# yuhang1008/WildGS-SLAM-Blackwell

Measured on AMD Instinct MI355X. Metric: rasterised Gaussians/s fwd+bwd @1M pts 1080p; PSNR vs ref, higher is better.
Workload: dtype f32; 1 GPU; configs[2]: 1000000 Gaussians, 1920x1080, SH3, single-view fwd+bwd, pose grad on; gaussians=1000000, image=1920x1080, sh_degree=3, num_rendered=13015374, parallelism=dp1 (keyframe views), dp_exchange=none

## Files before the change

wildgs-slam-blackwell_amd/csrc/capi.hip:

```cpp
#include <cstdarg>
#include <cstdio>
#include <cstdlib>
#include <cstring>
#include <vector>

#include <immintrin.h>

#include "wgsr.h"
#include "wgsr_common.h"
#include "wgsr_internal.h"

namespace wgsr {

namespace {
thread_local char g_err[1024] = "";

struct HostCounters {
  uint32_t* buf = nullptr;
  hipEvent_t ev = nullptr;
  hipStream_t side = nullptr;
  hipEvent_t pre = nullptr;
  uint4* mbox = nullptr;
  uint32_t seq = 0;
};
constexpr int kMaxDevices = 64;
int device_slot() {
  int dev = 0;
  return hipGetDevice(&dev) == hipSuccess && dev >= 0 && dev < kMaxDevices ? dev : -1;
}
struct BinningGuess {
  int P = -1, W = 0, H = 0, bshift = -1;
  size_t bytes = 0;
};
BinningGuess& binning_guess() {
  thread_local BinningGuess g[kMaxDevices];
  const int dev = device_slot();
  return g[dev < 0 ? 0 : dev];
}

bool publish_counts() {
  static const bool on = [] {
    const char* e = getenv("WGSR_PUBLISH_COUNTS");
    return !(e && e[0] == '0');
  }();
  return on;
}

HostCounters& host_counters() {
  thread_local HostCounters per_dev[kMaxDevices];
  const int dev = device_slot();
  HostCounters& hc = per_dev[dev < 0 ? 0 : dev];
  if (!hc.buf) {
    void* p = nullptr;
    if (hipHostMalloc(&p, kCounterBytes, hipHostMallocDefault) != hipSuccess) p = nullptr;
    hc.buf = static_cast<uint32_t*>(p);
    if (hipEventCreateWithFlags(&hc.ev, hipEventDisableTiming) != hipSuccess) hc.ev = nullptr;
    if (hipStreamCreateWithFlags(&hc.side, hipStreamNonBlocking) != hipSuccess) hc.side = nullptr;
    if (hc.side && hipEventCreateWithFlags(&hc.pre, hipEventDisableTiming) != hipSuccess) hc.pre = nullptr;
    if (!hc.pre) hc.side = nullptr;
    void* m = nullptr;
    if (publish_counts() &&
        hipHostMalloc(&m, 256, hipHostMallocCoherent | hipHostMallocMapped) == hipSuccess) {
      hc.mbox = static_cast<uint4*>(m);
      *hc.mbox = make_uint4(0u, 0u, 0u, 0u);
    }
  }
  return hc;
}

struct DevCounters {
  uint32_t* buf = nullptr;
  int parity = 0;
  bool failed = false;
};
bool bds_emit(int bshift) { return bshift <= 1; }

DevCounters* dev_counters(hipStream_t s) {
  thread_local DevCounters per_dev[kMaxDevices];
  const int dev = device_slot();
  if (dev < 0) return nullptr;
  DevCounters& dc = per_dev[dev];
  if (!dc.buf && !dc.failed) {
    void* p = nullptr;
    if (hipMalloc(&p, 2 * kCounterBytes) != hipSuccess || hipMemsetAsync(p, 0, 2 * kCounterBytes, s) != hipSuccess) {
      dc.failed = true;
      return nullptr;
    }
    dc.buf = static_cast<uint32_t*>(p);
  }
  return dc.buf ? &dc : nullptr;
}

}

int set_error(int code, const char* fmt, ...) {
  va_list ap;
  va_start(ap, fmt);
  vsnprintf(g_err, sizeof(g_err), fmt, ap);
  va_end(ap);
  return code;
}

int num_bits(uint32_t n) {
  int b = 0;
  while (b < 32 && (1ull << b) < n) ++b;
  return b;
}

namespace {

enum Stage { kStPreprocess, kStDepthSort, kStOffsetsScan, kStDuplicate, kStTileSort, kStRanges, kStRenderFwd,
             kStRenderBwd, kStGaussBwd, kStDistCuda2, kNumStages };
const char* const kStageNames[] = {"preprocess", "depth_sort", "offsets_scan", "duplicate", "tile_sort",
                                   "ranges",     "render_fwd", "render_bwd",   "gauss_bwd", "dist_cuda2"};
static_assert(kNumStages == WGSR_NUM_STAGES && sizeof(kStageNames) / sizeof(kStageNames[0]) == kNumStages,
              "Stage, kStageNames and WGSR_NUM_STAGES list the same stages in the same order");
struct Prof {
  uint32_t mask = 0;
  struct Rec { int stage; hipEvent_t a, b; };
  std::vector<Rec> recs;
  std::vector<hipEvent_t> pool;
  double ms[WGSR_NUM_STAGES] = {};
  int64_t count[WGSR_NUM_STAGES] = {};
  hipEvent_t get() {
    if (!pool.empty()) { hipEvent_t e = pool.back(); pool.pop_back(); return e; }
    hipEvent_t e = nullptr;
    if (hipEventCreate(&e) != hipSuccess) return nullptr;
    return e;
  }
  void flush() {
    for (auto& r : recs) {
      float t = 0.f;
      if (hipEventSynchronize(r.b) == hipSuccess && hipEventElapsedTime(&t, r.a, r.b) == hipSuccess) {
        ms[r.stage] += t;
        count[r.stage] += 1;
      }
      pool.push_back(r.a);
      pool.push_back(r.b);
    }
    recs.clear();
  }
};
Prof g_prof;

struct StageTimer {
  Stage stage;
  hipStream_t s;
  hipEvent_t a = nullptr;
  StageTimer(Stage st, hipStream_t str) : stage(st), s(str) {
    if (((g_prof.mask >> st) & 1u) && (a = g_prof.get()) && hipEventRecord(a, s) != hipSuccess) a = nullptr;
  }
  ~StageTimer() {
    if (!a) return;
    hipEvent_t b = g_prof.get();
    if (b && hipEventRecord(b, s) == hipSuccess) g_prof.recs.push_back({stage, a, b});
    else g_prof.pool.push_back(a);
  }
};

struct Grid {
  int gx, gy, nt;
  explicit Grid(const wgsr_raster_args& a)
      : gx((a.W + kTile - 1) / kTile), gy((a.H + kTile - 1) / kTile), nt(gx * gy) {}
};

int sort_bits(int n) { return num_bits((uint32_t)n) > 0 ? num_bits((uint32_t)n) : 1; }

constexpr int kDefaultBinShift = 2;
constexpr int kSmallFrameTiles = 2048;
int bin_shift(const wgsr_raster_args& a) {
  const char* e = getenv("WGSR_BIN_SHIFT");
  const Grid g(a);
  int sh = e ? atoi(e) : (g.nt <= kSmallFrameTiles ? 1 : kDefaultBinShift);
  sh = sh < 0 ? 0 : (sh > kMaxBinShift ? kMaxBinShift : sh);
  return sh > 0 && g.nt > 65535 ? 0 : sh;
}
enum class DepthSched { kBins, kGlobal, kFull };
DepthSched depth_schedule(int bshift) {
  const char* e = getenv("WGSR_DEPTH_SORT");
  if (e && strcmp(e, "full") == 0) return DepthSched::kFull;
  if (!bshift || (e && strcmp(e, "global") == 0)) return DepthSched::kGlobal;
  return DepthSched::kBins;
}
size_t bin_depth_max_avg() {
  const char* e = getenv("WGSR_BIN_DEPTH_MAX_AVG");
  return e ? (size_t)strtoull(e, nullptr, 10) : (size_t)6144;
}
constexpr int kDepthBits = 32;
constexpr bool kFullDepthInAlt = ((kDepthBits + 7) / 8) % 2 == 1;
thread_local int64_t g_depth_order_off = -1;

int validate(const wgsr_raster_args* a) {
  if (!a) return set_error(WGSR_EINVAL, "null args");
  if (a->P < 0) return set_error(WGSR_EINVAL, "means3D must have dimensions (num_points, 3)");
  if (a->W <= 0 || a->H <= 0) return set_error(WGSR_EINVAL, "image size must be positive (got %dx%d)", a->W, a->H);
  if (a->P == 0) return WGSR_OK;
  if (!a->means3D || !a->opacities || !a->bg || !a->viewmatrix || !a->projmatrix || !a->campos)
    return set_error(WGSR_EINVAL, "missing required tensor");
  if ((a->shs == nullptr) == (a->colors == nullptr))
    return set_error(WGSR_EINVAL, "Please provide excatly one of either SHs or precomputed colors!");
  const bool sr = a->scales && a->rotations;
  if (sr == (a->cov3D_precomp != nullptr))
    return set_error(WGSR_EINVAL,
                     "Please provide exactly one of either scale/rotation pair or precomputed 3D covariance!");
  if (a->shs && (a->M <= 0 || a->D < 0 || a->D > 3 || (a->D + 1) * (a->D + 1) > a->M))
    return set_error(WGSR_EINVAL, "invalid SH configuration (degree %d, %d coefficients)", a->D, a->M);
  const Grid g(*a);
  if (g.gx > 65535 || g.gy > 65535) return set_error(WGSR_EINVAL, "image too large");
  return WGSR_OK;
}

#define HIPCHK(expr)                                                                          \
  do {                                                                                        \
    hipError_t _e = (expr);                                                                   \
    if (_e != hipSuccess) return set_error(WGSR_EHIP, "%s: %s", #expr, hipGetErrorString(_e)); \
  } while (0)

#define STAGE(a, s, expr)                   \
  do {                                      \
    HIPCHK(expr);                           \
    if ((a).debug) {                        \
      HIPCHK(hipStreamSynchronize(s));      \
      HIPCHK(hipGetLastError());            \
    }                                       \
  } while (0)

void* call_alloc(wgsr_alloc_fn fn, void* ctx, size_t bytes) { return fn ? fn(ctx, bytes) : nullptr; }

struct Fwd {
  const wgsr_raster_args& a;
  hipStream_t s;
  Grid grid; GeomLayout GL; ImageLayout IL;
  int bshift;
  float *out_color, *out_depth, *out_opacity;
  int32_t* n_touched;
  void *geom = nullptr, *image = nullptr;
  uint32_t* counter = nullptr;
  template <typename T> T* g(size_t off) const { return at<T>(geom, off); }
  template <typename T> T* im(size_t off) const { return at<T>(image, off); }
  int alloc(wgsr_alloc_fn geom_alloc, wgsr_alloc_fn image_alloc, void* ctx) {
    if (!(geom = call_alloc(geom_alloc, ctx, GL.total)))
      return set_error(WGSR_EALLOC, "geometry buffer allocation failed");
    if (!(image = call_alloc(image_alloc, ctx, IL.total)))
      return set_error(WGSR_EALLOC, "image buffer allocation failed");
    return WGSR_OK;
  }
};

struct BinningPlan {
  BinLayout BL;
  size_t lists_bytes, bds_bytes, total;
  BinningPlan(size_t N_rect, size_t N_bin, int bshift, bool bin_depth)
      : BL(N_rect), lists_bytes(bshift ? align256(4 * (N_bin << (2 * bshift))) : 0),
        bds_bytes(bin_depth ? align256(16 * N_bin) : 0), total(BL.total + lists_bytes + bds_bytes) {}
};

struct Counts {
  size_t N_rect, N, N_bin;
  uint32_t flags;
  bool published;
};

int start_counts_readback(const Fwd& f, bool bin_depth, HostCounters& hc, PublishJob* pub) {
  if (!hc.buf || !hc.ev) return set_error(WGSR_EHIP, "pinned counter buffer / event allocation failed");
  if (bin_depth && hc.mbox) {
    *pub = PublishJob{f.counter, hc.mbox, hc.seq = (hc.seq % 0xFFFFFFu) + 1u};
  } else if (hc.side && !bin_depth) {
    HIPCHK(hipEventRecord(hc.pre, f.s));
    HIPCHK(hipStreamWaitEvent(hc.side, hc.pre, 0));
    HIPCHK(hipMemcpyAsync(hc.buf, f.counter, kCounterBytes, hipMemcpyDeviceToHost, hc.side));
    HIPCHK(hipEventRecord(hc.ev, hc.side));
  } else {
    HIPCHK(hipMemcpyAsync(hc.buf, f.counter, kCounterBytes, hipMemcpyDeviceToHost, f.s));
    HIPCHK(hipEventRecord(hc.ev, f.s));
  }
  return WGSR_OK;
}

int wait_counts(const Fwd& f, HostCounters& hc, const PublishJob& pub, Counts* c) {
  if (!pub.counter) {
    HIPCHK(hipEventSynchronize(hc.ev));
  } else {
    uint4 rec = make_uint4(0u, 0u, 0u, 0u);
    auto poll = [&]() {
      asm volatile("" ::: "memory");
      const __m128i v = _mm_load_si128(reinterpret_cast<const __m128i*>(const_cast<const uint4*>(hc.mbox)));
      _mm_storeu_si128(reinterpret_cast<__m128i*>(&rec), v);
      return (rec.x >> 8) == pub.seq;
    };
    uint32_t polls = 0;
    while (!poll()) {
      _mm_pause();
      if ((++polls & 1023u) == 0) {
        const hipError_t q = hipStreamQuery(f.s);
        if (q == hipErrorNotReady) continue;
        HIPCHK(q);
        bool seen = false;
        for (int k = 0; k < (1 << 16) && !(seen = poll()); ++k) _mm_pause();
        if (seen) break;
        hc.mbox = nullptr;
        break;
      }
    }
    if (hc.mbox && !(rec.x & 0x80u)) {
      *c = Counts{rec.y, rec.z, rec.w, rec.x & 0x7Fu, true};
      return WGSR_OK;
    }
    HIPCHK(hipMemcpyAsync(hc.buf, f.counter, kCounterBytes, hipMemcpyDeviceToHost, f.s));
    HIPCHK(hipStreamSynchronize(f.s));
  }
  *c = Counts{0, 0, 0, hc.buf[1], false};
  const uint64_t* partial = reinterpret_cast<const uint64_t*>(hc.buf + 4);
  for (int i = 0; i < kRectPairLanes; ++i) {
    c->N_rect += partial[i];
    c->N += partial[kRectPairLanes + i];
    c->N_bin += partial[2 * kRectPairLanes + i];
  }
  return WGSR_OK;
}

int read_depth_range(const Fwd& f, HostCounters& hc, const Counts& c, uint32_t* hi, uint32_t* nlo) {
  if (c.published) {
    HIPCHK(hipMemcpyAsync(hc.buf, f.counter, kCounterBytes, hipMemcpyDeviceToHost, f.s));
    HIPCHK(hipStreamSynchronize(f.s));
  }
  const uint32_t* rw = hc.buf + kDepthRangeOffset / 4;
  *hi = *nlo = 0;
  for (int i = 0; i < kRectPairLanes; ++i) {
    *hi = rw[i] > *hi ? rw[i] : *hi;
    *nlo = rw[kRectPairLanes + i] > *nlo ? rw[kRectPairLanes + i] : *nlo;
  }
  return WGSR_OK;
}

ZeroJob preprocess_zero_job(const Fwd& f, const DevCounters* dc, DepthSched sched) {
  const size_t P = (size_t)f.a.P;
  ZeroJob zj{};
  auto add = [&](void* p, size_t words) {
    if (words) { zj.p[zj.count] = static_cast<float*>(p); zj.n[zj.count++] = words; }
  };
  if (dc) add(dc->buf + (size_t)(dc->parity ^ 1) * (kCounterBytes / 4), kCounterBytes / 4);
  size_t sup_off = depth_sort_sup_offset_words(P);
  const size_t sup_words = sched == DepthSched::kFull     ? sort_sup_words(P, 0, kDepthBits, &sup_off)
                           : sched == DepthSched::kGlobal ? depth_sort_sup_words(P)
                                                          : 0;
  add(f.g<uint32_t>(f.GL.hist) + sup_off, sup_words);
  if (f.bshift) add(f.g<float>(f.GL.bsup), 2 * kScanSupStride * packed_scan_supers(P));
  return zj;
}

int queue_depth_sort(const Fwd& f, bool full, bool zero_sup, const uint32_t** depth_order) {
  const GeomLayout& GL = f.GL;
  const size_t P = (size_t)f.a.P;
  uint32_t *dkey = f.g<uint32_t>(GL.dkey), *dkey_alt = f.g<uint32_t>(GL.dkey_alt), *dval = f.g<uint32_t>(GL.dval),
           *dval_alt = f.g<uint32_t>(GL.dval_alt), *hist = f.g<uint32_t>(GL.hist);
  StageTimer T(kStDepthSort, f.s);
  if (full) {
    const bool sup_zeroed = sort_sup_words(P, 0, kDepthBits, nullptr) != 0;
    bool in_alt = false;
    STAGE(f.a, f.s, radix_sort_pairs(dkey, dkey_alt, dval, dval_alt, true, P, 0, kDepthBits, hist,
                                     f.g<uint32_t>(GL.totals), f.s, &in_alt, nullptr, nullptr, sup_zeroed));
    if (in_alt != kFullDepthInAlt) return set_error(WGSR_EHIP, "internal: depth sort parity");
    *depth_order = kFullDepthInAlt ? dval_alt : dval;
    return WGSR_OK;
  }
  if (zero_sup)
    HIPCHK(hipMemsetAsync(hist + depth_sort_sup_offset_words(P), 0, 4 * depth_sort_sup_words(P), f.s));
  STAGE(f.a, f.s, launch_depth_sort(dkey, dkey_alt, dval, dval_alt, P, f.counter + kDepthRangeOffset / 4,
                                    f.counter + 2, hist, f.s));
  *depth_order = dval_alt;
  return WGSR_OK;
}

int queue_scan(const Fwd& f, const uint32_t* depth_order, const PublishJob& pj) {
  const GeomLayout& GL = f.GL;
  StageTimer T(kStOffsetsScan, f.s);
  if (f.bshift) {
    STAGE(f.a, f.s, packed_scan_blocks(f.g<uint32_t>(GL.tb), 1, depth_order, (size_t)f.a.P, f.g<uint32_t>(GL.bsum),
// ... 454 lines not shown
```

wildgs-slam-blackwell_amd/csrc/raster_fwd.hip:

```cpp
#include <stdlib.h>
#include <string.h>

#include <type_traits>

#include "wgsr_common.h"
#include "wgsr_internal.h"

namespace wgsr {

namespace {

constexpr float SH_C0 = 0.28209479177387814f;
constexpr float SH_C1 = 0.4886025119029199f;
__constant__ float SH_C2[5] = {1.0925484305920792f, -1.0925484305920792f, 0.31539156525252005f,
                               -1.0925484305920792f, 0.5462742152960396f};
__constant__ float SH_C3[7] = {-0.5900435899266435f, 2.890611442640554f, -0.4570457994644658f,
                               0.3731763325901154f,  -0.4570457994644658f, 1.445305721320277f,
                               -0.5900435899266435f};

__device__ __forceinline__ f3 ldc(const float* sh, int k) { return mk3(sh[3 * k], sh[3 * k + 1], sh[3 * k + 2]); }

__device__ __forceinline__ f3 sh_to_rgb(int deg, const float* sh, f3 dir, uint32_t& clamp_bits) {
#pragma clang fp contract(off)
  auto term = [](float c, const float* v) -> f3 { return {c * v[0], c * v[1], c * v[2]}; };
// ... 350 lines not shown
      rg.ok = __shfl(rr.ok, lo, 64);
      for (int row = y0 + nt; !found && row < y1; ++row) {
        int xa;
        const uint32_t len = (uint32_t)row_span(rg, row, x0, x1, xa);
        if (local < acc + len) {
          ty = (uint32_t)row;
          tx = (uint32_t)xa + (local - acc);
          found = true;
        }
        acc += len;
      }
    }
    if (k < end) {
      keys[k] = ty * (uint32_t)gx + tx;
      slot_g[k] = gg;
      pflag[k] = 0;
    }
  }
}

__device__ __forceinline__ uint32_t bin_mask(int bx, int by, int bshift, int x0, int y0, int x1, int y1,
                                             const uint4& tab, bool tall, const Reach& rg) {
  const int B = 1 << bshift;
  const bool use_tab = x1 - x0 <= 255;
  uint32_t mask = 0;
  for (int rr = 0; rr < B; ++rr) {
    const int ty = (by << bshift) + rr;
    if (ty < y0 || ty >= y1) continue;
    const int kr = ty - y0;
    int xa, len;
    if (!tall || (use_tab && kr < kRowTab)) {
      xa = x0 + (int)rowtab_x(tab, kr);
      len = (int)rowtab_len(tab, kr);
    } else {
      len = row_span(rg, ty, x0, x1, xa);
    }
    const int cl = max(xa, bx << bshift), ch = min(xa + len, (bx << bshift) + B);
    if (ch > cl) mask |= ((1u << (ch - cl)) - 1u) << (rr * B + (cl - (bx << bshift)));
  }
  return mask;
}

template <int S>
__device__ __forceinline__ uint32_t bin_mask_tab(int bx, int by, int x0, int y0, const uint4& tab) {
  constexpr int B = 1 << S;
  const int kr0 = (by << S) - y0;
  const uint64_t L64 = ((uint64_t)tab.y << 32) | tab.x, X64 = ((uint64_t)tab.w << 32) | tab.z;
  const uint32_t sr = 8u * (uint32_t)max(kr0, 0), sl = 8u * (uint32_t)max(-kr0, 0);
  const uint32_t lens = (uint32_t)((L64 >> sr) << sl);
  const uint32_t xs = (uint32_t)((X64 >> sr) << sl);
  const int d0 = x0 - (bx << S);
  uint32_t mask = 0;
#pragma unroll
  for (int rr = 0; rr < B; ++rr) {
    const int xa = d0 + (int)((xs >> (8 * rr)) & 0xFFu);
    const int xe = xa + (int)((lens >> (8 * rr)) & 0xFFu);
    const int lo = min(max(xa, 0), B), hi = min(max(xe, 0), B);
    mask |= (((1u << hi) - 1u) ^ ((1u << lo) - 1u)) << (rr * B);
  }
  return mask;
}

constexpr int kDupScanThreads = kPackedScanTile;
template <int S>
__global__ __launch_bounds__(kDupScanThreads) void k_duplicate_bins(
    uint32_t P, int gbx, const ListRec* __restrict__ lrec, const uint32_t* __restrict__ sorted_g,
    const uint2* __restrict__ bsum, const uint2* __restrict__ bsup, const float4* __restrict__ splat,
    uint32_t* __restrict__ slot_start, uint8_t* __restrict__ pflag, uint32_t* __restrict__ keys,
    uint32_t* __restrict__ vals, const ZeroJob zero, uint32_t* __restrict__ meta, uint32_t cap_slots,
    uint32_t cap_pairs) {
  constexpr int NW = kDupScanThreads / 64;
  constexpr int bshift = S;
  __shared__ uint2 s_w[NW], s_p[NW];
  __shared__ uint4 s_ra[NW][64];
  __shared__ uint4 s_rt[NW][64];
  __shared__ uint2 s_rw[NW][64];
  __shared__ uint32_t s_own[NW][64];
  const int t = threadIdx.x, w = t >> 6, lane = t & 63;
  const uint32_t r = blockIdx.x * kDupScanThreads + t;
  const bool in = r < P;
  if (blockIdx.x == 0 && t == 0) meta[2] = sorted_g ? 0u : 1u;
  const uint32_t rc = min(r, P - 1u);
  const uint32_t g0 = sorted_g ? sorted_g[rc] : rc;
  uint4 lw = lrec[g0].w, tab = lrec[g0].tab;
  uint2 pre = make_uint2(0u, 0u);
  if (bsup) {
    const uint32_t b = blockIdx.x, sb = b / kScanSupBlocks;
    for (uint32_t q = (uint32_t)t; q < sb; q += kDupScanThreads) {
      const uint2 x = bsup[(size_t)q * kScanSupStride];
      pre.x += x.x;
      pre.y += x.y;
    }
    if ((uint32_t)t < kScanSupBlocks && sb * kScanSupBlocks + t < b) {
      const uint2 x = bsum[sb * kScanSupBlocks + t];
      pre.x += x.x;
      pre.y += x.y;
    }
  } else {
    pre = bsum[blockIdx.x];
  }
  const uint32_t g = in ? g0 : 0u;
  if (!in) {
    lw = make_uint4(0u, 0u, 0u, 0u);
    tab = lw;
  }
  const uint32_t v = lw.z;
  const uint32_t cnt = v & 0xFFFFu, nb = v >> 16;
  uint32_t rlo = 0, rhi = 0;
  bool tall = false;
  if (nb) {
    const ushort4 rc = lr_rect(lw);
    rlo = lw.x;
    rhi = lw.y;
    tall = rc.w - rc.y > kRowTab || !rowtab_ok(rc);
  } else {
    tab = make_uint4(0u, 0u, 0u, 0u);
  }
  const uint32_t ic = wave_incl_scan(cnt), ib = wave_incl_scan(nb);
  if (lane == 63) s_w[w] = make_uint2(ic, ib);
  uint2 wb;
  if (bsup) {
    pre.x = wave_sum_u32(pre.x);
    pre.y = wave_sum_u32(pre.y);
    if (lane == 0) s_p[w] = pre;
    __syncthreads();
    wb = make_uint2(0u, 0u);
#pragma unroll
    for (int k = 0; k < NW; ++k) {
      wb.x += s_p[k].x;
      wb.y += s_p[k].y;
    }
  } else {
    __syncthreads();
    wb = pre;
  }
#pragma unroll
  for (int k = 0; k < NW; ++k) {
    const uint2 x = s_w[k];
    if (k < w) { wb.x += x.x; wb.y += x.y; }
  }
  const uint2 wt = s_w[w];
  if (in) slot_start[g] = wb.x + ic - cnt;
  {
    const uint32_t f0 = wb.x, f1 = min(wb.x + wt.x, cap_slots);
    const uint32_t a0 = min((f0 + 3u) & ~3u, max(f1, f0)), a1 = max(f1 & ~3u, a0);
    if (lane < (int)(a0 - f0)) pflag[f0 + lane] = 0;
    if (lane < (int)(f1 - a1)) pflag[a1 + lane] = 0;
    uint32_t* pw = reinterpret_cast<uint32_t*>(pflag);
    for (uint32_t k = (a0 >> 2) + lane; k < (a1 >> 2); k += 64) pw[k] = 0u;
  }
  zero_share(zero, blockIdx.x, gridDim.x, t, kDupScanThreads);
  if (wt.y == 0) return;
  const uint32_t my_off = wb.y + ib - nb;
  const uint32_t start = wb.y, end = wb.y + wt.y;
  const bool any_tall = wave_any(tall);
  Reach rr{};
  if (any_tall && tall) rr = reach_of(splat[3 * (size_t)g], splat[3 * (size_t)g + 1]);
  s_ra[w][lane] = make_uint4(rlo, rhi, my_off, g);
  s_rt[w][lane] = tab;
  {
    const int bw = (((int)(rhi & 0xFFFFu) - 1) >> bshift) - ((int)(rlo & 0xFFFFu) >> bshift) + 1;
    s_rw[w][lane] = make_uint2((uint32_t)bw, __float_as_uint(__builtin_amdgcn_rcpf((float)bw)));
  }
  uint32_t carry = 0;
  for (uint32_t base = start; base < end; base += 64) {
    const uint32_t k = base + lane;
    const uint32_t kk = min(k, end - 1);
    s_own[w][lane] = lane == 0 ? carry : 0u;
    __builtin_amdgcn_wave_barrier();
    if (nb && my_off >= base && my_off < base + 64) s_own[w][my_off - base] = (uint32_t)lane;
    __builtin_amdgcn_wave_barrier();
    const uint32_t lo = wave_incl_max(s_own[w][lane]);
    carry = (uint32_t)__builtin_amdgcn_readlane((int)lo, 63);
    const uint4 ra = s_ra[w][lo];
    const uint32_t local = kk - ra.z;
    const uint32_t gg = ra.w;
    const int x0 = (int)(ra.x & 0xFFFFu), y0 = (int)(ra.x >> 16), x1 = (int)(ra.y & 0xFFFFu), y1 = (int)(ra.y >> 16);
    const uint4 tq = s_rt[w][lo];
    const uint2 rw = s_rw[w][lo];
    const int bx0 = x0 >> bshift, bw = (int)rw.x;
    int row = (int)((float)local * __uint_as_float(rw.y));
    int col = (int)local - row * bw;
    {
      const int dn = col < 0 ? 1 : 0, up = col >= bw ? 1 : 0;
      row += up - dn;
      col += (dn - up) * bw;
    }
    const int bx = bx0 + col, by = (y0 >> bshift) + row;
    uint32_t mask;
    if (!any_tall) {
      mask = bin_mask_tab<S>(bx, by, x0, y0, tq);
    } else {
      const bool tl = __shfl((int)tall, (int)lo, 64) != 0;
      Reach rg;
      rg.mx = __shfl(rr.mx, lo, 64); rg.my = __shfl(rr.my, lo, 64); rg.ca = __shfl(rr.ca, lo, 64);
      rg.cb = __shfl(rr.cb, lo, 64); rg.L = __shfl(rr.L, lo, 64); rg.det = __shfl(rr.det, lo, 64);
      rg.ey = __shfl(rr.ey, lo, 64); rg.dya = __shfl(rr.dya, lo, 64); rg.ica = __shfl(rr.ica, lo, 64);
      rg.ok = __shfl(rr.ok, lo, 64);
      mask = tl ? bin_mask(bx, by, bshift, x0, y0, x1, y1, tq, true, rg) : bin_mask_tab<S>(bx, by, x0, y0, tq);
    }
    if (k < end && k < cap_pairs) {
      keys[k] = (uint32_t)(by * gbx + bx) | (mask << 16);
      vals[k] = gg;
    }
    __builtin_amdgcn_wave_barrier();
  }
}

__global__ __launch_bounds__(256) void k_bin_bounds(const uint32_t* __restrict__ skeys, uint32_t NB,
                                                    uint2* __restrict__ bounds) {
  const uint32_t e = blockIdx.x * blockDim.x + threadIdx.x;
  if (e >= NB) return;
  const uint32_t b = skeys[e] & 0xFFFFu;
  if (e == 0 || (skeys[e - 1] & 0xFFFFu) != b) bounds[b].x = e;
  if (e + 1 == NB || (skeys[e + 1] & 0xFFFFu) != b) bounds[b].y = e + 1;
}

constexpr int kExpThreads = 256;
__global__ __launch_bounds__(kExpThreads) void k_expand_bins(const uint32_t* __restrict__ skeys,
                                                             const uint32_t* __restrict__ sgid,
                                                             const uint2* __restrict__ bounds, int gx, int gy,
                                                             int bshift, int gbx, uint32_t* __restrict__ lists,
                                                             uint2* __restrict__ ranges,
                                                             uint32_t* __restrict__ tile_len,
                                                             uint32_t* __restrict__ meta) {
  constexpr int NW = kExpThreads / 64;
  const int t = threadIdx.x, w = t >> 6, lane = t & 63;
  if (blockIdx.x == 0 && t == 0) meta[0] = 1u;
  const int B = 1 << bshift;
  const uint32_t bin = blockIdx.x >> bshift;
  const int r = (int)(blockIdx.x & (uint32_t)(B - 1));
  const int bx = (int)(bin % (uint32_t)gbx), by = (int)(bin / (uint32_t)gbx);
  const int ty = (by << bshift) + r;
  if (ty >= gy) return;
  const uint2 bb = bounds[bin];
  const uint32_t lo = bb.x, hi = bb.y, len = hi - lo;
  const size_t base0 = ((size_t)lo << (2 * bshift)) + (size_t)(r << bshift) * len;
  const uint32_t shift = 16u + ((uint32_t)r << bshift), rmask = (1u << B) - 1u;
  uint32_t count[4] = {0u, 0u, 0u, 0u};
  __shared__ unsigned long long s_wp[2][NW];
  uint32_t* const out0 = lists + base0;
  uint32_t key = lo + t < hi ? skeys[lo + t] : 0u, gid = lo + t < hi ? sgid[lo + t] : 0u;
  asm volatile("" ::"v"(key), "v"(gid));
  int par = 0;
  for (uint32_t e0 = lo; e0 < hi; e0 += kExpThreads, par ^= 1) {
    const uint32_t bits = (key >> shift) & rmask, my_gid = gid;
    const uint32_t e1 = e0 + kExpThreads + t;
    key = e1 < hi ? skeys[e1] : 0u;
    gid = e1 < hi ? sgid[e1] : 0u;
    uint64_t m[4];
    unsigned long long packed = 0ull;
#pragma unroll
    for (int c = 0; c < 4; ++c) {
      m[c] = wave_ballot(c < B && ((bits >> c) & 1u));
      packed |= (unsigned long long)__popcll(m[c]) << (16 * c);
    }
    if (lane == 0) s_wp[par][w] = packed;
    __syncthreads();
    unsigned long long off = 0ull, tot = 0ull;
#pragma unroll
    for (int k = 0; k < NW; ++k) {
      const unsigned long long v = s_wp[par][k];
      off += k < w ? v : 0ull;
      tot += v;
    }
#pragma unroll
    for (int c = 0; c < 4; ++c) {
      if (c >= B) break;
      if ((bits >> c) & 1u)
        out0[(uint32_t)c * len + count[c] + (uint32_t)((off >> (16 * c)) & 0xFFFFull) + lanes_below(m[c])] = my_gid;
      count[c] += (uint32_t)((tot >> (16 * c)) & 0xFFFFull);
    }
    asm volatile("" ::"v"(key), "v"(gid));
  }
  if (t < B) {
    const int tx = (bx << bshift) + t;
    if (tx < gx) {
      const uint32_t tile = (uint32_t)ty * (uint32_t)gx + (uint32_t)tx;
      const size_t b0 = base0 + (size_t)t * len;
      uint32_t c = 0;
#pragma unroll
      for (int k = 0; k < 4; ++k) c = k == t ? count[k] : c;
      ranges[tile] = make_uint2((uint32_t)b0, (uint32_t)b0 + c);
      tile_len[tile] = c;
    }
  }
}

constexpr int kBdsThreads = 512, kBdsWaves = kBdsThreads / 64, kBdsItems = 10;
constexpr int kBdsCap = kBdsThreads * kBdsItems;
constexpr int kBdsMaxBits = 9, kBdsDigits = 1 << kBdsMaxBits;
static_assert(kBdsDigits <= kBdsThreads, "threads t < kBdsDigits own digit t");
__device__ __forceinline__ bool bds_owns_digit() { return (int)threadIdx.x < kBdsDigits; }

struct BdsLds {
  union {
    uint2 buf[kBdsCap];
    unsigned long long match[kBdsWaves][kBdsDigits];
  };
  uint32_t wcnt[kBdsWaves][kBdsDigits];
  uint32_t base[kBdsDigits];
  uint32_t tmp[kBdsWaves];
  uint32_t rng[2][kBdsWaves];
  uint32_t etot[kBdsWaves][16];
  uint32_t erun[16];
};

struct BdsEmit {
  uint32_t* __restrict__ lists;
  uint2* __restrict__ ranges;
  uint32_t* __restrict__ tile_len;
  uint32_t* __restrict__ meta;
  int gx, gy, bshift, gbx;
};

template <int JN>
__device__ __forceinline__ void bds_emit_chunk(BdsLds& L, const uint32_t (&m)[JN], const uint32_t (&g)[JN],
                                               uint32_t cnt, int NT, uint32_t* __restrict__ out, uint32_t n) {
  const int w = threadIdx.x >> 6, lane = threadIdx.x & 63;
  uint32_t mine = 0;
  static_for<0, JN>([&](auto J) {
    constexpr int j = decltype(J)::value;
    if ((uint32_t)(w * JN + j) * 64u < cnt) {
      const uint32_t mj = m[j];
#pragma unroll 1
      for (int k = 0; k < NT; ++k) {
        const uint64_t b = wave_ballot((mj >> k) & 1u);
        mine += lane == k ? (uint32_t)__popcll(b) : 0u;
      }
    }
  });
  if (lane < 16) L.etot[w][lane] = mine;
  __syncthreads();
  uint32_t pre = 0;
  if (lane < NT) {
    pre = L.erun[lane];
    for (int q = 0; q < w; ++q) pre += L.etot[q][lane];
  }
  static_for<0, JN>([&](auto J) {
    constexpr int j = decltype(J)::value;
    if ((uint32_t)(w * JN + j) * 64u < cnt) {
      const uint32_t mj = m[j], gj = g[j];
#pragma unroll 1
      for (int k = 0; k < NT; ++k) {
        const bool bit = (mj >> k) & 1u;
        const uint64_t b = wave_ballot(bit);
        if (b != 0) {
          const uint32_t base = (uint32_t)__builtin_amdgcn_readlane((int)pre, k);
          if (bit) out[(size_t)k * n + base + lanes_below(b)] = gj;
          pre += lane == k ? (uint32_t)__popcll(b) : 0u;
        }
      }
    }
  });
  __syncthreads();
  if (w == kBdsWaves - 1 && lane < NT) L.erun[lane] = pre;
  __syncthreads();
}

__device__ __forceinline__ void bds_emit_ranges(const BdsLds& L, const BdsEmit& E, uint32_t bin, uint32_t lo,
                                                uint32_t n) {
  const int t = threadIdx.x;
  const int B = 1 << E.bshift;
  if (bin == 0 && t == 0) E.meta[0] = 1u;
  if (t < B * B) {
    const int r = t >> E.bshift, c = t & (B - 1);
    const int bx = (int)(bin % (uint32_t)E.gbx), by = (int)(bin / (uint32_t)E.gbx);
    const int tx = (bx << E.bshift) + c, ty = (by << E.bshift) + r;
    if (tx < E.gx && ty < E.gy) {
      const uint32_t tile = (uint32_t)ty * (uint32_t)E.gx + (uint32_t)tx;
      const uint32_t b0 = (lo << (2 * E.bshift)) + (uint32_t)t * n;
      const uint32_t c_t = n ? L.erun[t] : 0u;
      E.ranges[tile] = make_uint2(b0, b0 + c_t);
      E.tile_len[tile] = c_t;
    }
  }
}

__device__ __forceinline__ uint32_t bds_excl_scan(uint32_t v, uint32_t* s_tmp, uint32_t* total) {
  const int w = threadIdx.x >> 6, lane = threadIdx.x & 63;
  const uint32_t inc = wave_incl_scan(v);
  if (lane == 63) s_tmp[w] = inc;
  __syncthreads();
  uint32_t base = 0, tot = 0;
#pragma unroll
  for (int i = 0; i < kBdsWaves; ++i) {
    const uint32_t x = s_tmp[i];
    base += i < w ? x : 0u;
    tot += x;
  }
  __syncthreads();
  *total = tot;
  return base + inc - v;
}

constexpr int kBdsPosBits = 13, kBdsRankShift = kBdsPosBits + kBdsMaxBits;
static_assert(kBdsCap <= (1 << kBdsPosBits) && kBdsItems * 64 <= (1 << (32 - kBdsRankShift)), "pk packing");
__device__ __forceinline__ uint32_t bds_digit(uint32_t pk) { return (pk >> kBdsPosBits) & (kBdsDigits - 1); }
template <int JN>
__device__ __forceinline__ void bds_rank(BdsLds& L, uint32_t cn, uint32_t mn, int shift, int bits,
                                         const uint32_t (&k)[JN], uint32_t (&pk)[JN]) {
  const int w = threadIdx.x >> 6, lane = threadIdx.x & 63;
  const uint32_t mask = (1u << bits) - 1u;
#pragma unroll
  for (int j = 0; j < JN; ++j) {
    const uint32_t le = (uint32_t)(w * JN + j) * 64u + (uint32_t)lane;
    const bool valid = le < cn;
    const uint32_t d = ((k[j] - mn) >> shift) & mask;
    (void)bits;
    if (valid) atomicOr(&L.match[w][d], 1ull << lane);
    const uint64_t peers = valid ? L.match[w][d] : 0ull;
    if (valid) L.match[w][d] = 0ull;
    const int leader = __ffsll((unsigned long long)peers) - 1;
    uint32_t old = 0;
    if (valid && lane == leader) old = atomicAdd(&L.wcnt[w][d], (uint32_t)__popcll(peers));
    old = (uint32_t)__shfl((int)old, leader & 63, 64);
    const uint32_t rk = old + lanes_below(peers);
    pk[j] = (pk[j] & ((1u << kBdsPosBits) - 1u)) | (d << kBdsPosBits) | (rk << kBdsRankShift);
    __builtin_amdgcn_sched_barrier(0);
  }
}
__device__ __forceinline__ uint32_t bds_slot(const BdsLds& L, uint32_t pk) {
  const int w = threadIdx.x >> 6;
  const uint32_t d = bds_digit(pk);
  return L.base[d] + L.wcnt[w][d] + (pk >> kBdsRankShift);
}

__device__ __forceinline__ uint32_t bds_wave_prefix(BdsLds& L) {
  const int t = threadIdx.x;
  uint32_t run = 0;
  if (!bds_owns_digit()) return 0u;
#pragma unroll
  for (int q = 0; q < kBdsWaves; ++q) {
    const uint32_t x = L.wcnt[q][t];
    L.wcnt[q][t] = run;
    run += x;
  }
  return run;
}

__device__ __forceinline__ uint2 bds_load_scratch(const uint2* p) { return *p; }

__device__ __forceinline__ uint32_t bds_range(BdsLds& L, uint32_t mn, uint32_t mx, int& R) {
  const int w = threadIdx.x >> 6, lane = threadIdx.x & 63;
#pragma unroll
  for (int off = 32; off >= 1; off >>= 1) {
    mn = min(mn, (uint32_t)__shfl_xor((int)mn, off, 64));
    mx = max(mx, (uint32_t)__shfl_xor((int)mx, off, 64));
  }
  if (lane == 0) {
    L.rng[0][w] = mn;
    L.rng[1][w] = mx;
  }
  __syncthreads();
#pragma unroll
  for (int q = 0; q < kBdsWaves; ++q) {
    mn = min(mn, L.rng[0][q]);
    mx = max(mx, L.rng[1][q]);
  }
  const uint32_t span = mx - mn;
  R = span ? 32 - __clz((int)span) : 0;
  return mn;
}
__device__ __forceinline__ void bds_plan(int R, int& passes, int& pbits) {
  passes = (R + kBdsMaxBits - 1) / kBdsMaxBits;
  pbits = passes ? (R + passes - 1) / passes : 0;
}

template <int JN>
__device__ __forceinline__ void bds_small(BdsLds& L, const uint32_t* __restrict__ skeys,
                                          const uint32_t* __restrict__ sgid, const uint32_t* __restrict__ sdep,
                                          const uint32_t* __restrict__ gdep, uint32_t lo, uint32_t n,
                                          uint32_t* __restrict__ okeys, uint32_t* __restrict__ ogid, bool E,
                                          const BdsEmit& EM) {
  const int t = threadIdx.x, w = t >> 6, lane = t & 63;
  constexpr uint32_t kPosMask = (1u << kBdsPosBits) - 1u;
  uint32_t k[JN], pk[JN];
  uint32_t mn = 0xFFFFFFFFu, mx = 0u;
  if (gdep) {
#pragma unroll
    for (int j = 0; j < JN; ++j) k[j] = sgid[lo + min((uint32_t)(w * JN + j) * 64u + (uint32_t)lane, n - 1u)];
#pragma unroll
    for (int j = 0; j < JN; ++j) k[j] = gdep[k[j]];
  } else {
#pragma unroll
    for (int j = 0; j < JN; ++j) k[j] = sdep[lo + min((uint32_t)(w * JN + j) * 64u + (uint32_t)lane, n - 1u)];
  }
#pragma unroll
  for (int j = 0; j < JN; ++j) {
    const uint32_t le = (uint32_t)(w * JN + j) * 64u + (uint32_t)lane;
    pk[j] = le;
    k[j] = le < n ? k[j] : 0u;
    if (le < n) {
      mn = min(mn, k[j]);
      mx = max(mx, k[j]);
    }
  }
  int R, npass, pbits;
  mn = bds_range(L, mn, mx, R);
  bds_plan(R, npass, pbits);
  for (int p = 0; p < npass; ++p) {
    const int shift = p * pbits, bits = min(pbits, R - shift);
    bds_rank<JN>(L, n, mn, shift, bits, k, pk);
    __syncthreads();
    uint32_t all;
    const uint32_t ex = bds_excl_scan(bds_wave_prefix(L), L.tmp, &all);
    if (bds_owns_digit()) L.base[t] = ex;
    __syncthreads();
#pragma unroll
    for (int j = 0; j < JN; ++j) {
      const uint32_t le = (uint32_t)(w * JN + j) * 64u + (uint32_t)lane;
      if (le < n) L.buf[bds_slot(L, pk[j])] = make_uint2(k[j], pk[j] & kPosMask);
    }
    __syncthreads();
#pragma unroll
    for (int j = 0; j < JN; ++j) {
      const uint32_t le = (uint32_t)(w * JN + j) * 64u + (uint32_t)lane;
      if (le < n) {
        const uint2 kv = L.buf[le];
        k[j] = kv.x;
        pk[j] = kv.y;
      }
    }
#pragma unroll
    for (int q = 0; q < kBdsWaves; ++q)
      if (bds_owns_digit()) L.wcnt[q][t] = 0u;
    if (p + 1 < npass) {
      __syncthreads();
      for (int i = t; i < kBdsWaves * kBdsDigits; i += kBdsThreads) (&L.match[0][0])[i] = 0ull;
    }
    __syncthreads();
  }
  if (E) {
    uint32_t m[JN], g[JN];
    const uint32_t tmask = (1u << (1 << (2 * EM.bshift))) - 1u;
#pragma unroll
    for (int j = 0; j < JN; ++j) {
      const uint32_t le = (uint32_t)(w * JN + j) * 64u + (uint32_t)lane;
      const uint32_t q = le < n ? pk[j] & kPosMask : 0u;
      m[j] = skeys[lo + q];
      g[j] = sgid[lo + q];
    }
#pragma unroll
    for (int j = 0; j < JN; ++j) {
      const uint32_t le = (uint32_t)(w * JN + j) * 64u + (uint32_t)lane;
      m[j] = le < n ? (m[j] >> 16) & tmask : 0u;
      g[j] = le < n ? g[j] : 0u;
    }
    if (t < 16) L.erun[t] = 0u;
    __syncthreads();
    bds_emit_chunk<JN>(L, m, g, n, 1 << (2 * EM.bshift), EM.lists + ((size_t)lo << (2 * EM.bshift)), n);
    return;
  }
  uint32_t ok[JN], og[JN];
#pragma unroll
  for (int j = 0; j < JN; ++j) {
    const uint32_t le = (uint32_t)(w * JN + j) * 64u + (uint32_t)lane;
    const uint32_t q = le < n ? pk[j] & kPosMask : 0u;
    pk[j] = q;
    ok[j] = okeys ? skeys[lo + q] : 0u;
    og[j] = sgid ? sgid[lo + q] : q;
  }
#pragma unroll
  for (int j = 0; j < JN; ++j) {
    const uint32_t le = (uint32_t)(w * JN + j) * 64u + (uint32_t)lane;
    if (le < n) {
      if (okeys) okeys[lo + le] = ok[j];
      ogid[lo + le] = og[j];
    }
  }
}

template <int JN>
__device__ __forceinline__ void bds_emit_big(BdsLds& L, const uint32_t* __restrict__ skeys,
                                             const uint32_t* __restrict__ sgid, const uint2* fin, uint32_t lo,
                                             uint32_t n, const BdsEmit& E) {
  const int t = threadIdx.x, w = t >> 6, lane = t & 63;
  const uint32_t tmask = (1u << (1 << (2 * E.bshift))) - 1u;
  constexpr uint32_t kChunk = JN * kBdsThreads;
  if (t < 16) L.erun[t] = 0u;
  __syncthreads();
  uint32_t* out = E.lists + ((size_t)lo << (2 * E.bshift));
  for (uint32_t c0 = 0; c0 < n; c0 += kChunk) {
    const uint32_t cn = min(kChunk, n - c0);
    uint32_t m[JN], g[JN];
#pragma unroll
    for (int j = 0; j < JN; ++j) {
      const uint32_t le = (uint32_t)(w * JN + j) * 64u + (uint32_t)lane;
      m[j] = 0u;
      g[j] = 0u;
      if (le < cn) {
        const uint32_t q = fin ? bds_load_scratch(fin + c0 + le).y : c0 + le;
        m[j] = (skeys[lo + q] >> 16) & tmask;
        g[j] = sgid[lo + q];
      }
    }
    bds_emit_chunk<JN>(L, m, g, cn, 1 << (2 * E.bshift), out, n);
  }
}

__device__ __forceinline__ void bds_big(BdsLds& L, const uint32_t* __restrict__ skeys, const uint32_t* __restrict__ sgid,
                                     const uint32_t* __restrict__ gdep, uint32_t lo, uint32_t n, uint32_t NL,
                                     uint32_t* __restrict__ okeys, uint32_t* __restrict__ ogid, uint2* scratch,
                                     bool E, const BdsEmit& EM) {
  const int t = threadIdx.x, w = t >> 6, lane = t & 63;
  uint32_t mn = 0xFFFFFFFFu, mx = 0u;
  auto dep = [&](uint32_t e) { return gdep[sgid[lo + e]]; };
  for (uint32_t e = (uint32_t)t; e < n; e += kBdsThreads) {
    const uint32_t x = dep(e);
    mn = min(mn, x);
    mx = max(mx, x);
  }
  int R, passes, pbits;
  mn = bds_range(L, mn, mx, R);
  bds_plan(R, passes, pbits);
  constexpr int JN = 7;
  if (passes == 0) {
    if (E) {
      bds_emit_big<JN>(L, skeys, sgid, nullptr, lo, n, EM);
      return;
    }
    for (uint32_t e = (uint32_t)t; e < n; e += kBdsThreads) {
      okeys[lo + e] = skeys[lo + e];
      ogid[lo + e] = sgid[lo + e];
    }
    return;
  }
  constexpr uint32_t kChunk = JN * kBdsThreads;
  uint2* bufA = scratch + lo;
  uint2* bufB = scratch + NL + lo;
  for (int p = 0; p < passes; ++p) {
    const int shift = p * pbits, bits = min(pbits, R - shift);
    const uint32_t mask = (1u << bits) - 1u;
    const uint2* src = (p & 1) ? bufA : bufB;
    uint2* dst = (p & 1) ? bufB : bufA;
    auto load = [&](uint32_t e) -> uint2 {
      return p == 0 ? make_uint2(dep(e), e) : bds_load_scratch(src + e);
    };
    if (bds_owns_digit()) L.base[t] = 0u;
    __syncthreads();
    for (uint32_t e = (uint32_t)t; e < n; e += kBdsThreads) atomicAdd(&L.base[((load(e).x - mn) >> shift) & mask], 1u);
    __syncthreads();
    {
      uint32_t all;
      const uint32_t c = bds_owns_digit() ? L.base[t] : 0u;
      const uint32_t ex = bds_excl_scan(c, L.tmp, &all);
      if (bds_owns_digit()) L.base[t] = ex;
    }
    __syncthreads();
    for (uint32_t c0 = 0; c0 < n; c0 += kChunk) {
      const uint32_t cn = min(kChunk, n - c0);
      uint32_t k[JN], pk[JN], pos[JN];
#pragma unroll
      for (int j = 0; j < JN; ++j) {
        const uint32_t le = (uint32_t)(w * JN + j) * 64u + (uint32_t)lane;
        k[j] = 0u;
        pos[j] = 0u;
        pk[j] = 0u;
        if (le < cn) {
          const uint2 kv = load(c0 + le);
          k[j] = kv.x;
          pos[j] = kv.y;
        }
      }
      bds_rank<JN>(L, cn, mn, shift, bits, k, pk);
      __syncthreads();
      const uint32_t tot = bds_wave_prefix(L);
      __syncthreads();
#pragma unroll
      for (int j = 0; j < JN; ++j) {
        const uint32_t le = (uint32_t)(w * JN + j) * 64u + (uint32_t)lane;
        if (le < cn) dst[bds_slot(L, pk[j])] = make_uint2(k[j], pos[j]);
      }
      __syncthreads();
      if (bds_owns_digit()) L.base[t] += tot;
#pragma unroll
      for (int q = 0; q < kBdsWaves; ++q)
        if (bds_owns_digit()) L.wcnt[q][t] = 0u;
      __syncthreads();
    }
    __syncthreads();
  }
  const uint2* fin = ((passes - 1) & 1) ? bufB : bufA;
  if (E) {
    bds_emit_big<JN>(L, skeys, sgid, fin, lo, n, EM);
    return;
  }
  for (uint32_t e = (uint32_t)t; e < n; e += kBdsThreads) {
    const uint32_t q = bds_load_scratch(fin + e).y;
    okeys[lo + e] = skeys[lo + q];
    ogid[lo + e] = sgid[lo + q];
  }
}

__global__ __launch_bounds__(kBdsThreads) void k_bin_depth_sort(
    const uint32_t* __restrict__ skeys, const uint32_t* __restrict__ sgid, const uint2* __restrict__ bounds,
    const uint32_t* __restrict__ gdep, uint32_t NL,
    uint32_t* __restrict__ okeys, uint32_t* __restrict__ ogid, uint2* scratch, BdsEmit emit) {
  __shared__ BdsLds L;
  const int t = threadIdx.x;
  const uint32_t bin = blockIdx.x;
  const uint2 bb = bounds[bin];
  const uint32_t lo = bb.x, n = bb.y - bb.x;
  const bool E = emit.lists != nullptr;
  if (n == 0) {
    if (E) bds_emit_ranges(L, emit, bin, lo, 0u);
    return;
  }
#pragma unroll
  for (int q = 0; q < kBdsWaves; ++q)
    if (bds_owns_digit()) L.wcnt[q][t] = 0u;
  for (int i = t; i < kBdsWaves * kBdsDigits; i += kBdsThreads) (&L.match[0][0])[i] = 0ull;
  if (n <= 1u * kBdsThreads)
    bds_small<1>(L, skeys, sgid, nullptr, gdep, lo, n, okeys, ogid, E, emit);
  else if (n <= 2u * kBdsThreads)
    bds_small<2>(L, skeys, sgid, nullptr, gdep, lo, n, okeys, ogid, E, emit);
  else if (n <= 3u * kBdsThreads)
    bds_small<3>(L, skeys, sgid, nullptr, gdep, lo, n, okeys, ogid, E, emit);
  else if (n <= 4u * kBdsThreads)
    bds_small<4>(L, skeys, sgid, nullptr, gdep, lo, n, okeys, ogid, E, emit);
  else if (n <= 5u * kBdsThreads)
    bds_small<5>(L, skeys, sgid, nullptr, gdep, lo, n, okeys, ogid, E, emit);
  else if (n <= 6u * kBdsThreads)
    bds_small<6>(L, skeys, sgid, nullptr, gdep, lo, n, okeys, ogid, E, emit);
  else if (n <= 7u * kBdsThreads)
    bds_small<7>(L, skeys, sgid, nullptr, gdep, lo, n, okeys, ogid, E, emit);
  else if (kBdsItems > 8 && n <= 8u * kBdsThreads)
    bds_small<(kBdsItems > 8 ? 8 : 7)>(L, skeys, sgid, nullptr, gdep, lo, n, okeys, ogid, E, emit);
  else if (kBdsItems > 9 && n <= 9u * kBdsThreads)
    bds_small<(kBdsItems > 9 ? 9 : 7)>(L, skeys, sgid, nullptr, gdep, lo, n, okeys, ogid, E, emit);
  else if (kBdsItems > 7 && n <= (uint32_t)kBdsCap)
    bds_small<kBdsItems>(L, skeys, sgid, nullptr, gdep, lo, n, okeys, ogid, E, emit);
  else
    bds_big(L, skeys, sgid, gdep, lo, n, NL, okeys, ogid, scratch, E, emit);
  if (E) bds_emit_ranges(L, emit, bin, lo, n);
}

constexpr int kOrderBuckets = 1024;

__device__ __forceinline__ void tile_chunk(uint32_t x, uint32_t nt, uint32_t& c0, uint32_t& c1) {
  const uint32_t q = nt / 8, r = nt % 8;
  c0 = x < r ? x * (q + 1) : r * (q + 1) + (x - r) * q;
  c1 = c0 + (x < r ? q + 1 : q);
}

__device__ __forceinline__ uint32_t tile_work(const uint32_t* __restrict__ work, bool quads, uint32_t tile) {
  if (!quads) return work[tile];
  const uint4 q = reinterpret_cast<const uint4*>(work)[tile];
  return max(max(q.x, q.y), max(q.z, q.w));
}

__device__ __forceinline__ void order_chunk(uint32_t c0, uint32_t c1, const uint32_t* __restrict__ work, bool quads,
                                            uint32_t* __restrict__ order, uint32_t* s_cnt) {
  const int t = threadIdx.x;
  s_cnt[t] = 0;
  __syncthreads();
  auto bucket = [&](uint32_t tile) {
    return (uint32_t)(kOrderBuckets - 1) - min((uint32_t)(kOrderBuckets - 1), tile_work(work, quads, tile));
  };
  for (uint32_t tile = c0 + t; tile < c1; tile += 1024) atomicAdd(&s_cnt[bucket(tile)], 1u);
  __syncthreads();
  __shared__ uint32_t s_w[16];
  const uint32_t v = s_cnt[t];
  uint32_t inc = v;
#pragma unroll
  for (int off = 1; off < 64; off <<= 1) {
    const uint32_t o = __shfl_up(inc, off, 64);
    if ((t & 63) >= off) inc += o;
  }
  if ((t & 63) == 63) s_w[t >> 6] = inc;
  __syncthreads();
  uint32_t base = 0;
  for (int i = 0; i < (t >> 6); ++i) base += s_w[i];
  __syncthreads();
  s_cnt[t] = base + inc - v;
  __syncthreads();
  for (uint32_t tile = c0 + t; tile < c1; tile += 1024) order[c0 + atomicAdd(&s_cnt[bucket(tile)], 1u)] = tile;
}

__global__ __launch_bounds__(256) void k_ranges(const uint32_t* __restrict__ keys, uint32_t N, int ntiles,
                                                uint2* __restrict__ ranges, uint32_t* __restrict__ len,
                                                uint32_t* __restrict__ meta) {
  const int t = blockIdx.x * blockDim.x + threadIdx.x;
  if (t == 0) meta[0] = 0u;
  if (t >= ntiles) return;
  auto lower = [&](uint32_t v) {
    uint32_t lo = 0, hi = N;
    while (lo < hi) {
      const uint32_t mid = (lo + hi) >> 1;
      if (keys[mid] < v) lo = mid + 1; else hi = mid;
    }
    return lo;
  };
  const uint2 r = make_uint2(lower((uint32_t)t), lower((uint32_t)t + 1));
  ranges[t] = r;
  len[t] = r.y - r.x;
}

__global__ __launch_bounds__(1024) void k_tile_order(const uint32_t* __restrict__ work, bool quads, bool global,
                                                     uint32_t ntiles, uint32_t* __restrict__ order) {
  __shared__ uint32_t s_cnt[kOrderBuckets];
  uint32_t c0 = 0, c1 = ntiles;
  if (!global) tile_chunk(blockIdx.x, ntiles, c0, c1);
  order_chunk(c0, c1, work, quads, order, s_cnt);
}

constexpr int kFwdBatch = 64;

struct FwdPairRec {
  float4 q[3];
  float4 c[2];
  uint32_t n[2];
  uint32_t pad[2];
};
struct FwdPairLds {
  FwdPairRec p[kFwdBatch / 2];
  uint32_t touch[kFwdBatch];
};

template <bool kTouch>
__device__ __forceinline__ void fwd_blend_one(float a, float pw, const float4& C, uint32_t cn, uint32_t* touch_slot,
                                              float& T, v2f& c01, v2f& c2d, uint32_t& last, uint64_t& dm,
                                              uint64_t valid) {
  const float test_T = fmaf(-T, a, T);
  const uint64_t live = wave_ballot(pw <= 0.0f) & wave_ballot(a >= kMinAlpha) & ~dm & valid;
  const uint64_t low = wave_ballot(test_T < kMinT);
  const uint64_t blend = live & ~low;
  const bool bl = __builtin_amdgcn_inverse_ballot_w64(blend);
  const float wgt = bl ? a * T : 0.f;
  c01 += wgt * v2f{C.x, C.y};
  c2d += wgt * v2f{C.z, C.w};
  uint32_t tot = 0;
  if (kTouch) tot = (uint32_t)__popcll(blend & wave_ballot(test_T > 0.5f));
  T = bl ? test_T : T;
  last = bl ? cn : last;
  dm |= live & low;
  if (kTouch) *touch_slot = tot;
}

template <bool kTouch>
__device__ __forceinline__ void fwd_blend_pairs(int n, const FwdPairLds& L, uint32_t* touch, v2f pxy, float& T,
                                                v2f& c01, v2f& c2d, uint32_t& last, uint64_t& dm) {
  for (int i = 0; i < n && dm != ~0ull; i += 2) {
    const FwdPairRec& R = L.p[i >> 1];
    const float4 q0 = R.q[0], q1 = R.q[1], q2 = R.q[2];
    const float4 C1 = R.c[0], C2 = R.c[1];
    const uint2 cn = *reinterpret_cast<const uint2*>(&R.n[0]);
    const v2f DX = v2f{q0.x, q0.y} - v2f{pxy.x, pxy.x}, DY = v2f{q0.z, q0.w} - v2f{pxy.y, pxy.y};
    const v2f tz = v2f{q1.x, q1.y} * DX, tw = v2f{q1.z, q1.w} * DY;
    const v2f PW = pfma(DX, pfma(v2f{q2.x, q2.y}, DY, tz), tw * DY);
    const v2f ag = v2f{q2.z, q2.w} * v2f{__builtin_amdgcn_exp2f(PW.x), __builtin_amdgcn_exp2f(PW.y)};
    const float a1 = fminf(kMaxAlpha, ag.x), a2 = fminf(kMaxAlpha, ag.y);
    fwd_blend_one<kTouch>(a1, PW.x, C1, cn.x, touch + i, T, c01, c2d, last, dm, ~0ull);
    fwd_blend_one<kTouch>(a2, PW.y, C2, cn.y, touch + i + 1, T, c01, c2d, last, dm, i + 1 < n ? ~0ull : 0ull);
  }
}

template <class F>
__device__ __forceinline__ void fwd_blend_batch_pairs(int cnt, uint32_t cbase, const float4* sA, const float4* sB,
                                                      const float4* sC, const uint32_t* sG, FwdPairLds& L, int wx0,
                                                      int wx1, int wy0, int wy1, v2f pxy, int lane,
                                                      int32_t* __restrict__ n_touched, float& T, v2f& c01, v2f& c2d,
                                                      uint32_t& last, uint64_t& dm, uint32_t* fl_gid,
                                                      uint32_t* fl_tv, const float4* pre, uint32_t pre_gid, F after) {
  const float4 A = pre ? pre[0] : sA[lane], B = pre ? pre[1] : sB[lane];
  const bool mine = lane < cnt && ellipse_hits(A, B, wx0, wx1, wy0, wy1);
  const uint64_t todo = wave_ballot(mine);
  const int n = __popcll(todo);
  const uint32_t k = lanes_below(todo);
  const bool touch = (wave_ballot(T > 0.5f) & ~dm) != 0;
  if (mine) {
    FwdPairRec& R = L.p[k >> 1];
    float* q = &R.q[0].x + (k & 1);
    q[0] = A.x; q[2] = A.y; q[4] = A.z; q[6] = A.w; q[8] = B.x; q[10] = B.y;
    R.c[k & 1] = pre ? pre[2] : sC[lane];
    R.n[k & 1] = cbase + (uint32_t)lane;
  }
  if (touch) L.touch[lane] = 0;
  if (lane == 63 && (n & 1)) {
    FwdPairRec& R = L.p[n >> 1];
    float* q = &R.q[0].x + 1;
    q[0] = 0.f; q[2] = 0.f; q[4] = 0.f; q[6] = 0.f; q[8] = 0.f; q[10] = 0.f;
    R.c[1] = make_float4(0.f, 0.f, 0.f, 0.f);
  }
  __builtin_amdgcn_wave_barrier();
  after();
  if (touch) {
    fwd_blend_pairs<true>(n, L, L.touch, pxy, T, c01, c2d, last, dm);
    const uint32_t tv = mine ? L.touch[k] : 0u;
    if (fl_tv) {
      *fl_gid = pre_gid;
      *fl_tv = tv;
    } else if (tv != 0) {
      atomicAdd(&n_touched[sG[lane]], (int)tv);
    }
  } else {
    fwd_blend_pairs<false>(n, L, L.touch, pxy, T, c01, c2d, last, dm);
  }
  __builtin_amdgcn_wave_barrier();
}
// ... 489 lines not shown
```

Measured before the change: 1.409 billion Gaussians/s.

## Restructure binned-tile emit as per-wave tile walk through LDS staging

Measured after the change: 1.434 billion Gaussians/s, median of 6. 1.8% higher.

```diff
diff --git a/wildgs-slam-blackwell_amd/csrc/capi.hip b/wildgs-slam-blackwell_amd/csrc/capi.hip
--- a/wildgs-slam-blackwell_amd/csrc/capi.hip
+++ b/wildgs-slam-blackwell_amd/csrc/capi.hip
@@ -73,7 +73,7 @@
   int parity = 0;
   bool failed = false;
 };
-bool bds_emit(int bshift) { return bshift <= 1; }
+bool bds_emit(int bshift) { return bshift >= 1 && bshift <= kMaxBinShift; }
 
 DevCounters* dev_counters(hipStream_t s) {
   thread_local DevCounters per_dev[kMaxDevices];
diff --git a/wildgs-slam-blackwell_amd/csrc/raster_fwd.hip b/wildgs-slam-blackwell_amd/csrc/raster_fwd.hip
--- a/wildgs-slam-blackwell_amd/csrc/raster_fwd.hip
+++ b/wildgs-slam-blackwell_amd/csrc/raster_fwd.hip
@@ -676,8 +676,7 @@
   uint32_t base[kBdsDigits];
   uint32_t tmp[kBdsWaves];
   uint32_t rng[2][kBdsWaves];
-  uint32_t etot[kBdsWaves][16];
-  uint32_t erun[16];
+  uint32_t ecnt[16];
 };
 
 struct BdsEmit {
@@ -688,47 +687,69 @@
   int gx, gy, bshift, gbx;
 };
 
+template <int TPW>
+__device__ __forceinline__ void bds_emit_walk(BdsLds& L, uint32_t cnt, uint32_t* __restrict__ out, uint32_t n,
+                                              uint32_t (&run)[2]) {
+  static_assert(TPW == 1 || TPW == 2, "16 or 4 tiles over eight waves");
+  const uint32_t lane = threadIdx.x & 63u;
+  const uint32_t w = (uint32_t)__builtin_amdgcn_readfirstlane((int)(threadIdx.x >> 6));
+  const uint32_t groups = (cnt + 63u) >> 6;
+  const uint32_t k0 = TPW == 2 ? w : (w & 3u);
+  uint32_t g0 = 0u, g1 = groups;
+  if (TPW == 1) {
+    const uint32_t h = (groups + 1u) >> 1;
+    if (w >> 2) g0 = h; else g1 = h;
+  }
+  uint32_t kbit[TPW];
+  uint32_t* dst[TPW];
+#pragma unroll
+  for (int i = 0; i < TPW; ++i) {
+    const uint32_t k = k0 + 8u * (uint32_t)i;
+    kbit[i] = 1u << k;
+    dst[i] = out + (size_t)k * n + run[i];
+  }
+  auto emit = [&](const uint2 e, uint32_t g) {
+    const bool st = TPW == 2 || (g >= g0 && g < g1);
+#pragma unroll
+    for (int i = 0; i < TPW; ++i) {
+      const bool bit = (e.x & kbit[i]) != 0u;
+      const uint64_t b = wave_ballot(bit);
+      if (st && bit) dst[i][lanes_below(b)] = e.y;
+      dst[i] += __popcll(b);
+    }
+  };
+  const uint2* src = L.buf + lane;
+  uint2 ea = src[0], eb;
+  uint32_t g = 0;
+  for (; g + 1u < groups; g += 2u) {
+    eb = src[(g + 1u) * 64u];
+    emit(ea, g);
+    if (g + 2u < groups) ea = src[(g + 2u) * 64u];
+    emit(eb, g + 1u);
+  }
+  if (g < groups) emit(ea, g);
+#pragma unroll
+  for (int i = 0; i < TPW; ++i) {
+    const uint32_t k = k0 + 8u * (uint32_t)i;
+    run[i] = (uint32_t)(dst[i] - (out + (size_t)k * n));
+    if (lane == 0u && (TPW == 2 || w < 4u)) L.ecnt[k] = run[i];
+  }
+}
+
 template <int JN>
 __device__ __forceinline__ void bds_emit_chunk(BdsLds& L, const uint32_t (&m)[JN], const uint32_t (&g)[JN],
-                                               uint32_t cnt, int NT, uint32_t* __restrict__ out, uint32_t n) {
+                                               uint32_t cnt, int NT, uint32_t* __restrict__ out, uint32_t n,
+                                               uint32_t (&run)[2]) {
   const int w = threadIdx.x >> 6, lane = threadIdx.x & 63;
-  uint32_t mine = 0;
-  static_for<0, JN>([&](auto J) {
-    constexpr int j = decltype(J)::value;
-    if ((uint32_t)(w * JN + j) * 64u < cnt) {
-      const uint32_t mj = m[j];
-#pragma unroll 1
-      for (int k = 0; k < NT; ++k) {
-        const uint64_t b = wave_ballot((mj >> k) & 1u);
-        mine += lane == k ? (uint32_t)__popcll(b) : 0u;
-      }
-    }
-  });
-  if (lane < 16) L.etot[w][lane] = mine;
+#pragma unroll
+  for (int j = 0; j < JN; ++j)
+    if ((uint32_t)(w * JN + j) * 64u < cnt)
+      L.buf[(uint32_t)(w * JN + j) * 64u + (uint32_t)lane] = make_uint2(m[j], g[j]);
   __syncthreads();
-  uint32_t pre = 0;
-  if (lane < NT) {
-    pre = L.erun[lane];
-    for (int q = 0; q < w; ++q) pre += L.etot[q][lane];
-  }
-  static_for<0, JN>([&](auto J) {
-    constexpr int j = decltype(J)::value;
-    if ((uint32_t)(w * JN + j) * 64u < cnt) {
-      const uint32_t mj = m[j], gj = g[j];
-#pragma unroll 1
-      for (int k = 0; k < NT; ++k) {
-        const bool bit = (mj >> k) & 1u;
-        const uint64_t b = wave_ballot(bit);
-        if (b != 0) {
-          const uint32_t base = (uint32_t)__builtin_amdgcn_readlane((int)pre, k);
-          if (bit) out[(size_t)k * n + base + lanes_below(b)] = gj;
-          pre += lane == k ? (uint32_t)__popcll(b) : 0u;
-        }
-      }
-    }
-  });
-  __syncthreads();
-  if (w == kBdsWaves - 1 && lane < NT) L.erun[lane] = pre;
+  if (NT == 16)
+    bds_emit_walk<2>(L, cnt, out, n, run);
+  else
+    bds_emit_walk<1>(L, cnt, out, n, run);
   __syncthreads();
 }
 
@@ -744,7 +765,7 @@
     if (tx < E.gx && ty < E.gy) {
       const uint32_t tile = (uint32_t)ty * (uint32_t)E.gx + (uint32_t)tx;
       const uint32_t b0 = (lo << (2 * E.bshift)) + (uint32_t)t * n;
-      const uint32_t c_t = n ? L.erun[t] : 0u;
+      const uint32_t c_t = n ? L.ecnt[t] : 0u;
       E.ranges[tile] = make_uint2(b0, b0 + c_t);
       E.tile_len[tile] = c_t;
     }
@@ -921,9 +942,8 @@
       m[j] = le < n ? (m[j] >> 16) & tmask : 0u;
       g[j] = le < n ? g[j] : 0u;
     }
-    if (t < 16) L.erun[t] = 0u;
-    __syncthreads();
-    bds_emit_chunk<JN>(L, m, g, n, 1 << (2 * EM.bshift), EM.lists + ((size_t)lo << (2 * EM.bshift)), n);
+    uint32_t run[2] = {0u, 0u};
+    bds_emit_chunk<JN>(L, m, g, n, 1 << (2 * EM.bshift), EM.lists + ((size_t)lo << (2 * EM.bshift)), n, run);
     return;
   }
   uint32_t ok[JN], og[JN];
@@ -949,27 +969,32 @@
 __device__ __forceinline__ void bds_emit_big(BdsLds& L, const uint32_t* __restrict__ skeys,
                                              const uint32_t* __restrict__ sgid, const uint2* fin, uint32_t lo,
                                              uint32_t n, const BdsEmit& E) {
-  const int t = threadIdx.x, w = t >> 6, lane = t & 63;
+  const int w = threadIdx.x >> 6, lane = threadIdx.x & 63;
   const uint32_t tmask = (1u << (1 << (2 * E.bshift))) - 1u;
   constexpr uint32_t kChunk = JN * kBdsThreads;
-  if (t < 16) L.erun[t] = 0u;
-  __syncthreads();
   uint32_t* out = E.lists + ((size_t)lo << (2 * E.bshift));
+  uint32_t run[2] = {0u, 0u};
   for (uint32_t c0 = 0; c0 < n; c0 += kChunk) {
     const uint32_t cn = min(kChunk, n - c0);
     uint32_t m[JN], g[JN];
 #pragma unroll
+    for (int j = 0; j < JN; ++j) g[j] = c0 + min((uint32_t)(w * JN + j) * 64u + (uint32_t)lane, cn - 1u);
+    if (fin) {
+#pragma unroll
+      for (int j = 0; j < JN; ++j) g[j] = bds_load_scratch(fin + g[j]).y;
+    }
+#pragma unroll
+    for (int j = 0; j < JN; ++j) {
+      m[j] = skeys[lo + g[j]];
+      g[j] = sgid[lo + g[j]];
+    }
+#pragma unroll
     for (int j = 0; j < JN; ++j) {
       const uint32_t le = (uint32_t)(w * JN + j) * 64u + (uint32_t)lane;
-      m[j] = 0u;
-      g[j] = 0u;
-      if (le < cn) {
-        const uint32_t q = fin ? bds_load_scratch(fin + c0 + le).y : c0 + le;
-        m[j] = (skeys[lo + q] >> 16) & tmask;
-        g[j] = sgid[lo + q];
-      }
-    }
-    bds_emit_chunk<JN>(L, m, g, cn, 1 << (2 * E.bshift), out, n);
+      m[j] = le < cn ? (m[j] >> 16) & tmask : 0u;
+      g[j] = le < cn ? g[j] : 0u;
+    }
+    bds_emit_chunk<JN>(L, m, g, cn, 1 << (2 * E.bshift), out, n, run);
   }
 }
 
```
